# Labbeti/conette-audio-captioning

Hardware: AMD Instinct MI355X
Metric: clips_per_sec (higher is better)
Workload: dtype bf16; 1 GPU; B=64/GPU x 10 s @ 32 kHz clips, ConvNeXt encoder + beam-3 KV-cached decode (min 3 / max 20 tokens, V=5631), synthetic seeded checkpoint; batch_per_gpu=64, global_batch=64, beam_size=3, parallelism=dp1, world_size_observed=1, allreduce_of_ones=1, decode_group=2, decode_streams=2, encode_streams=1, input_batches_rotated=4

## Files before the change

conette-audio-captioning_amd/csrc/encoder.hip:

```cpp
#include <stddef.h>

#include "ctx.h"
#include <type_traits>
#include <utility>

__device__ int g_cn_nonfinite;
__device__ __forceinline__ void cn_watch_stat(float v) {
  if (!(__builtin_fabsf(v) <= 3.0e38f)) atomicAdd(&g_cn_nonfinite, 1);
}

#include "gemm2.h"
#include "mlp_rc2.h"
#include "mlp_rs16.h"
#include "mlp_sp.h"
#include "down_fused.h"
#include "enc_tags.h"

template <typename XT>
__global__ __launch_bounds__(256) void cn_stem_mfma_kernel(const float* __restrict__ in, int F, int H0, long n_pos,
                                                           const float* __restrict__ w , const float* __restrict__ bias,
                                                           const float* __restrict__ ln_w, const float* __restrict__ ln_b,
                                                           XT* __restrict__ out) {
  __shared__ __attribute__((aligned(16))) float s_p[3 * 96];
  for (int i = threadIdx.x; i < 3 * 96; i += 256) s_p[i] = i < 96 ? bias[i] : i < 192 ? ln_w[i - 96] : ln_b[i - 192];
  const int lane = threadIdx.x & 63, j = lane & 31, h = lane >> 5;
  float a[3][8];
#pragma unroll
  for (int t = 0; t < 3; ++t)
#pragma unroll
    for (int s = 0; s < 8; ++s) a[t][s] = w[(4 * (s >> 1) + 2 * h + (s & 1)) * 96 + 32 * t + cn_rc2_chan(j)];
  __syncthreads();
  const long n_tiles = (n_pos + 31) >> 5;
  const long n_waves = (long)gridDim.x * 4;
  for (long tile = (long)blockIdx.x * 4 + (threadIdx.x >> 6); tile < n_tiles; tile += n_waves) {
    const long pos = tile * 32 + j;
    const long p = pos < n_pos ? pos : n_pos - 1;
    const int wq = (int)(p % 56);
    const long tt = p / 56;
    const int hh = (int)(tt % H0);
    const int b = (int)(tt / H0);
    f32x2 xv[4];
#pragma unroll
    for (int i = 0; i < 4; ++i) {
      const int r = 4 * hh - 4 + i;
      xv[i] = f32x2{0.f, 0.f};
      if (r >= 0 && r < F) xv[i] = *(const f32x2*)(in + ((size_t)b * F + r) * CN_N_MELS + 4 * wq + 2 * h);
    }
    f32x16 acc[3];
#pragma unroll
    for (int t = 0; t < 3; ++t)
#pragma unroll
      for (int u = 0; u < 2; ++u) {
        const f32x4 b0 = *(const f32x4*)(s_p + 32 * t + 16 * u + 8 * h), b1 = *(const f32x4*)(s_p + 32 * t + 16 * u + 8 * h + 4);
#pragma unroll
        for (int e = 0; e < 4; ++e) acc[t][8 * u + e] = b0[e], acc[t][8 * u + 4 + e] = b1[e];
      }
#pragma unroll
    for (int s = 0; s < 8; ++s)
#pragma unroll
      for (int t = 0; t < 3; ++t) acc[t] = __builtin_amdgcn_mfma_f32_32x32x2f32(a[t][s], xv[s >> 1][s & 1], acc[t], 0, 0, 0);
    float sum = 0.f;
#pragma unroll
    for (int t = 0; t < 3; ++t)
#pragma unroll
      for (int r = 0; r < 16; ++r) sum += acc[t][r];
    sum += __shfl_xor(sum, 32);
    const float mean = sum * (1.0f / 96.0f);
    float v2 = 0.f;
#pragma unroll
    for (int t = 0; t < 3; ++t)
#pragma unroll
      for (int r = 0; r < 16; ++r) {
        acc[t][r] -= mean;
        v2 = fmaf(acc[t][r], acc[t][r], v2);
      }
    v2 += __shfl_xor(v2, 32);
    const float rstd = 1.0f / sqrtf(v2 * (1.0f / 96.0f) + 1e-6f);
    if (pos < n_pos) {
      XT* o = out + (size_t)pos * 96 + 8 * h;
#pragma unroll
      for (int t = 0; t < 3; ++t)
#pragma unroll
        for (int u = 0; u < 2; ++u) {
          const int ch = 32 * t + 16 * u + 8 * h;
          float v[8];
#pragma unroll
          for (int q = 0; q < 2; ++q) {
            const f32x4 lw = *(const f32x4*)(s_p + 96 + ch + 4 * q), lb = *(const f32x4*)(s_p + 192 + ch + 4 * q);
#pragma unroll
            for (int e = 0; e < 4; ++e) v[4 * q + e] = acc[t][8 * u + 4 * q + e] * rstd * lw[e] + lb[e];
          }
          if constexpr (sizeof(XT) == 2) {
            *(cn_h8<XT>*)(o + 32 * t + 16 * u) = cn_h8<XT>{cn_from_f32<XT>(v[0]), cn_from_f32<XT>(v[1]), cn_from_f32<XT>(v[2]), cn_from_f32<XT>(v[3]),
                                                          cn_from_f32<XT>(v[4]), cn_from_f32<XT>(v[5]), cn_from_f32<XT>(v[6]), cn_from_f32<XT>(v[7])};
          } else {
            *(f32x4*)(o + 32 * t + 16 * u) = f32x4{v[0], v[1], v[2], v[3]};
            *(f32x4*)(o + 32 * t + 16 * u + 4) = f32x4{v[4], v[5], v[6], v[7]};
          }
        }
    }
  }
}

__device__ unsigned long long g_dw_prof[8];
#define DW_STAMP(i)                                                   \
  if (dbg) {                                                          \
    const unsigned long long t_ = clock64();                          \
    if ((threadIdx.x & 63) == 0) atomicAdd(&g_dw_prof[i], t_ - t_prev); \
    t_prev = t_;                                                      \
  }

template <int C, int S, int TH> struct DwTile {
  static constexpr int NCHUNK = C / 4;
  static constexpr int PITCH4 = NCHUNK | 1;
  static constexpr int PITCH = PITCH4 * 4;
};

template <int... U, typename F> __device__ __forceinline__ void cn_static_for(std::integer_sequence<int, U...>, F&& f) {
  (f(std::integral_constant<int, U>{}), ...);
}
__device__ __forceinline__ void cn_dw_pin1(float& v) { asm volatile("" : "+v"(v) : : "memory"); }
template <int TH, size_t... I> __device__ __forceinline__ void cn_dw_pin(float (&acc)[TH][4], std::index_sequence<I...>) {
  (cn_dw_pin1(acc[I / 4][I % 4]), ...);
}
__device__ __forceinline__ void cn_dw_opaque(unsigned& v) { asm volatile("" : "+v"(v)); }

template <typename T, typename XT, int C, int S, int TH, bool CLAMPED = false>
__global__ __launch_bounds__((C > 384 ? 384 : C) * S) void cn_dwconv_ln_kernel(const XT* __restrict__ x, int H, int W, int tiles_h,
                                                            int tiles_w, const float* __restrict__ dw_w ,
                                                            const unsigned* __restrict__ dw_wp ,
                                                            const float* __restrict__ dw_b,
                                                            const float* __restrict__ ln_w,
                                                            const float* __restrict__ ln_b, T* __restrict__ y,
                                                            int dbg) {
  extern __shared__ __attribute__((aligned(16))) char smem_raw[];
  float* s_v = (float*)smem_raw;
  unsigned long long t_prev = dbg ? clock64() : 0;
  constexpr int NP = TH * 4;
  constexpr int CT = C > 384 ? 384 : C;
  constexpr int PITCH = DwTile<C, S, TH>::PITCH;
  const int tid = threadIdx.x;
  const int c0 = tid % CT, sidx = tid / CT;
  int bid = cn_xcd_remap(blockIdx.x, gridDim.x);
  const int tw = bid % tiles_w;
  bid /= tiles_w;
  const int th = bid % tiles_h;
  const int b = bid / tiles_h;
  const int h0 = th * TH, w0 = tw * (4 * S) + sidx * 4;

  int wcl[10];
  bool wok[10];
#pragma unroll
  for (int q = 0; q < 10; ++q) {
    const int ww = w0 - 3 + q;
    wok[q] = (ww >= 0) && (ww < W);
    wcl[q] = min(max(ww, 0), W - 1) * C;
  }
#pragma unroll 1
  for (int c = c0; c < C; c += CT) {
  float acc[TH][4];
  const float bias = dw_b[c];
#pragma unroll
  for (int a = 0; a < TH; ++a)
#pragma unroll
    for (int e = 0; e < 4; ++e) acc[a][e] = bias;
  const XT* xb = x + (size_t)b * H * W * C + c;
  const bool interior = (h0 >= 3) && (h0 + TH + 3 <= H) && (w0 >= 3) && (w0 + 4 + 3 <= W);
  if constexpr (sizeof(XT) == 2) {
    static_assert(TH % 2 == 0, "row pairs");
    cn_h2 ke[3][7], ko[3][7];
#pragma unroll
    for (int a = 0; a < 3; ++a)
#pragma unroll
      for (int j = 0; j < 7; ++j) {
        ke[a][j] = __builtin_bit_cast(cn_h2, dw_wp[(a * 7 + j) * C + c]);
        ko[a][j] = __builtin_bit_cast(cn_h2, dw_wp[(21 + a * 7 + j) * C + c]);
      }
    DW_STAMP(0)
    auto fma_pair = [&](int r, const cn_h2 (&p)[10]) {
#pragma unroll
      for (int oh = 0; oh < TH; ++oh) {
        const int i = r - oh;
        if (i < -1 || i > 6) continue;
#pragma unroll
        for (int q = 0; q < 10; ++q)
#pragma unroll
          for (int ow = 0; ow < 4; ++ow) {
            const int j = q - ow;
            if (j < 0 || j > 6) continue;
            if (i == -1) acc[oh][ow] = fmaf((float)p[q][1], (float)ke[0][j][0], acc[oh][ow]);
            else if (i == 6) acc[oh][ow] = fmaf((float)p[q][0], (float)ko[2][j][1], acc[oh][ow]);
            else if ((i & 1) == 0) acc[oh][ow] = __builtin_amdgcn_fdot2(p[q], ke[i >> 1][j], acc[oh][ow], false);
            else acc[oh][ow] = __builtin_amdgcn_fdot2(p[q], ko[i >> 1][j], acc[oh][ow], false);
          }
      }
    };
    constexpr int NPR = (TH + 6) / 2;
    if constexpr (!CLAMPED) {
      const bool left = (w0 == 0), right = (w0 + 7 > W);
      const unsigned oL = 2u * (unsigned)((left ? 0 : w0 - 3) * C + c), oM = 2u * (unsigned)(w0 * C + c);
      const unsigned oR = 2u * (unsigned)((right ? w0 + 1 : w0 + 4) * C + c);
      constexpr unsigned SEL_PAIR = 0x05040100u, SEL_ZERO = 0x0c0c0c0cu;
      const unsigned selL = left ? SEL_ZERO : SEL_PAIR, selR = right ? SEL_ZERO : SEL_PAIR;
      const char* xc = (const char*)(x + (size_t)b * H * W * C);
      const bool rows_in = (h0 >= 3) && (h0 + TH + 3 <= H);
      const unsigned rows = ((1u << min(TH + 6, H + 3 - h0)) - 1u) & ~((1u << max(0, 3 - h0)) - 1u);
      auto conv = [&](auto check_rows) {
        constexpr bool CHECK = decltype(check_rows)::value;
        auto load_row = [&](int r, unsigned (&v)[10]) {
          const int hh = h0 - 3 + r;
          if (!CHECK || ((rows >> r) & 1u)) {
            const char* xr = xc + (size_t)hh * W * C * 2;
#pragma unroll
            for (int q = 0; q < 10; ++q)
              v[q] = *(const unsigned short*)(q < 3 ? xr + (size_t)oL + q * C * 2 : q < 7 ? xr + (size_t)oM + (q - 3) * C * 2 : xr + (size_t)oR + (q - 7) * C * 2);
          } else {
#pragma unroll
            for (int q = 0; q < 10; ++q) v[q] = 0u;
          }
        };
        auto pack = [&](const unsigned (&v0)[10], const unsigned (&v1)[10], cn_h2 (&p)[10]) {
#pragma unroll
          for (int q = 0; q < 10; ++q)
            p[q] = __builtin_bit_cast(cn_h2, __builtin_amdgcn_perm(v1[q], v0[q], q < 3 ? selL : q < 7 ? SEL_PAIR : selR));
        };
        auto pin = [&]() {
          if constexpr (CHECK) cn_dw_pin(acc, std::make_index_sequence<TH * 4>{});
        };
        unsigned a0[10], a1[10], b0[10], b1[10];
        cn_h2 p[10];
        load_row(0, a0);
        load_row(1, a1);
        cn_static_for(std::make_integer_sequence<int, (NPR + 1) / 2>{}, [&](auto k) {
          constexpr int u = 2 * decltype(k)::value;
          if (u + 1 < NPR) {
            load_row(2 * u + 2, b0);
            load_row(2 * u + 3, b1);
          }
          pack(a0, a1, p);
          fma_pair(2 * u, p);
          pin();
          if (u + 2 < NPR) {
            load_row(2 * u + 4, a0);
            load_row(2 * u + 5, a1);
          }
          if (u + 1 < NPR) {
            pack(b0, b1, p);
            fma_pair(2 * (u + 1), p);
            pin();
          }
        });
      };
      if (rows_in) conv(std::false_type{});
      else conv(std::true_type{});
    } else {
#pragma unroll
      for (int u = 0; u < NPR; ++u) {
        const int hh0 = h0 - 3 + 2 * u, hh1 = hh0 + 1;
        const bool ok0 = (hh0 >= 0) && (hh0 < H), ok1 = (hh1 >= 0) && (hh1 < H);
        const XT* x0 = xb + (size_t)min(max(hh0, 0), H - 1) * W * C;
        const XT* x1 = xb + (size_t)min(max(hh1, 0), H - 1) * W * C;
        XT v0[10], v1[10];
#pragma unroll
        for (int q = 0; q < 10; ++q) v0[q] = x0[wcl[q]], v1[q] = x1[wcl[q]];
        cn_h2 p[10];
#pragma unroll
        for (int q = 0; q < 10; ++q) p[q] = cn_h2{(ok0 && wok[q]) ? v0[q] : (XT)0.f, (ok1 && wok[q]) ? v1[q] : (XT)0.f};
        fma_pair(2 * u, p);
      }
    }
  } else {
  float k[49];
#pragma unroll
  for (int i = 0; i < 49; ++i) k[i] = dw_w[i * C + c];
  DW_STAMP(0)
  auto fma_row = [&](int r, const XT (&v)[10]) {
#pragma unroll
    for (int oh = 0; oh < TH; ++oh) {
      const int i = r - oh;
      if (i < 0 || i > 6) continue;
#pragma unroll
      for (int q = 0; q < 10; ++q)
#pragma unroll
        for (int ow = 0; ow < 4; ++ow) {
          const int j = q - ow;
          if (j < 0 || j > 6) continue;
          acc[oh][ow] = fmaf((float)v[q], k[i * 7 + j], acc[oh][ow]);
        }
    }
  };
  if (interior) {
    const XT* base = xb + ((size_t)(h0 - 3) * W + (w0 - 3)) * C;
    XT va[10], vb[10];
#pragma unroll
    for (int q = 0; q < 10; ++q) va[q] = base[q * C];
#pragma unroll
    for (int r = 0; r < TH + 6; r += 2) {
      if (r + 1 < TH + 6) {
        const XT* xr = base + (size_t)(r + 1) * W * C;
#pragma unroll
        for (int q = 0; q < 10; ++q) vb[q] = xr[q * C];
      }
      fma_row(r, va);
      if (r + 2 < TH + 6) {
        const XT* xr = base + (size_t)(r + 2) * W * C;
#pragma unroll
        for (int q = 0; q < 10; ++q) va[q] = xr[q * C];
      }
      if (r + 1 < TH + 6) fma_row(r + 1, vb);
    }
  } else {
#pragma unroll
    for (int r = 0; r < TH + 6; ++r) {
      const int hh = h0 - 3 + r;
      const bool hok = (hh >= 0) && (hh < H);
      const XT* xr = xb + (size_t)min(max(hh, 0), H - 1) * W * C;
      XT v[10];
#pragma unroll
      for (int q = 0; q < 10; ++q) v[q] = xr[wcl[q]];
#pragma unroll
      for (int q = 0; q < 10; ++q) v[q] = (hok && wok[q]) ? v[q] : (XT)0.f;
      fma_row(r, v);
    }
  }
  }
#pragma unroll
  for (int oh = 0; oh < TH; ++oh)
#pragma unroll
    for (int ow = 0; ow < 4; ++ow) s_v[((sidx * NP) + oh * 4 + ow) * PITCH + c] = acc[oh][ow];
  DW_STAMP(1)
  }
  __syncthreads();
  DW_STAMP(2)

  constexpr int NPOS = NP * S, NT = CT * S, PARTS = NT / NPOS, NCHUNK = C / 4, CPT = NCHUNK / PARTS;
  static_assert(NT % NPOS == 0 && NCHUNK % PARTS == 0, "LayerNorm thread mapping");
  float* s_ps = s_v + NPOS * PITCH;
  float* s_mean = s_ps + NPOS * PARTS;
  float* s_rstd = s_mean + NPOS;
  {
    const int pos = tid % NPOS, part = tid / NPOS;
    const float* row = s_v + pos * PITCH + part * 4;
    f32x4 seg[CPT];
    float sum = 0.f;
#pragma unroll
    for (int i = 0; i < CPT; ++i) {
      seg[i] = *(const f32x4*)(row + i * PARTS * 4);
      sum += (seg[i][0] + seg[i][1]) + (seg[i][2] + seg[i][3]);
    }
    s_ps[part * NPOS + pos] = sum;
    __syncthreads();
    float mean = 0.f;
#pragma unroll
    for (int j = 0; j < PARTS; ++j) mean += s_ps[j * NPOS + pos];
    mean *= (1.0f / C);
    float sq = 0.f;
#pragma unroll
    for (int i = 0; i < CPT; ++i)
#pragma unroll
      for (int e = 0; e < 4; ++e) {
        const float d = seg[i][e] - mean;
        sq = fmaf(d, d, sq);
      }
    __syncthreads();
    s_ps[part * NPOS + pos] = sq;
    __syncthreads();
    if (part == 0) {
      float var = 0.f;
#pragma unroll
      for (int j = 0; j < PARTS; ++j) var += s_ps[j * NPOS + pos];
      s_mean[pos] = mean;
      s_rstd[pos] = 1.0f / sqrtf(var * (1.0f / C) + 1e-6f);
      cn_watch_stat(var);
    }
    __syncthreads();
  }
  DW_STAMP(3)
  constexpr int C8 = C / 8;
  static_assert(NT % C8 == 0, "a thread keeps its 8 channels over all its items: the LN affine is loaded once");
  const int c8 = (tid % C8) * 8;
  const f32x4 lw0 = *(const f32x4*)(ln_w + c8), lw1 = *(const f32x4*)(ln_w + c8 + 4);
  const f32x4 lb0 = *(const f32x4*)(ln_b + c8), lb1 = *(const f32x4*)(ln_b + c8 + 4);
  for (int item = tid; item < NPOS * C8; item += NT) {
    const int pos = item / C8;
    const int ps = pos / NP, oh = (pos % NP) >> 2, ow = pos & 3;
    const int h = h0 + oh, w = tw * (4 * S) + ps * 4 + ow;
    if (h >= H || w >= W) continue;
    const float mean = s_mean[pos], rstd = s_rstd[pos];
    const f32x4 v0 = *(const f32x4*)(s_v + pos * PITCH + c8), v1 = *(const f32x4*)(s_v + pos * PITCH + c8 + 4);
    T* dst = y + (((size_t)b * H + h) * W + w) * C + c8;
    float o[8];
#pragma unroll
    for (int i = 0; i < 8; ++i) o[i] = ((i < 4 ? v0[i] : v1[i - 4]) - mean) * rstd * (i < 4 ? lw0[i] : lw1[i - 4]) + (i < 4 ? lb0[i] : lb1[i - 4]);
    cn_store8(dst, o);
  }
  DW_STAMP(4)
}

extern "C" int conette_debug_g2prof(unsigned long long* out16, int reset) {
  if (out16) CN_HIP(hipMemcpyFromSymbol(out16, HIP_SYMBOL(g_g2_prof), 128));
  if (reset) {
    unsigned long long z[16] = {0};
    CN_HIP(hipMemcpyToSymbol(HIP_SYMBOL(g_g2_prof), z, 128));
  }
// ... 253 lines not shown
      q1 = fmaf(a1[i] - m1, a1[i] - m1, q1);
    }
    q0 = cn_wave_sum_dpp(q0);
    q1 = cn_wave_sum_dpp(q1);
    if (lane == 0) {
      s_mean[p0] = m0;
      s_rstd[p0] = 1.0f / sqrtf(q0 * (1.0f / C) + 1e-6f);
      s_mean[p1] = m1;
      s_rstd[p1] = 1.0f / sqrtf(q1 * (1.0f / C) + 1e-6f);
      cn_watch_stat(q0 + q1);
    }
  }
  __syncthreads();
  constexpr int C8 = C / 8;
  static_assert(CT % C8 == 0, "a thread keeps its 8 channels over all its items: the LN affine is loaded once");
  const int c8 = (tid % C8) * 8;
  const f32x4 lw0 = *(const f32x4*)(ln_w + c8), lw1 = *(const f32x4*)(ln_w + c8 + 4);
  const f32x4 lb0 = *(const f32x4*)(ln_b + c8), lb1 = *(const f32x4*)(ln_b + c8 + 4);
  for (int item = tid; item < NPOS * C8; item += CT) {
    const int pos = item / C8;
    const int h = h0 + pos / WW, w = pos % WW;
    if (h >= H) continue;
    const float mean = s_mean[pos], rstd = s_rstd[pos];
    const f32x4 v0 = *(const f32x4*)(s_v + pos * PITCH + c8), v1 = *(const f32x4*)(s_v + pos * PITCH + c8 + 4);
    T* dst = y + (((size_t)b * H + h) * WW + w) * C + c8;
    float o[8];
#pragma unroll
    for (int i = 0; i < 8; ++i) o[i] = ((i < 4 ? v0[i] : v1[i - 4]) - mean) * rstd * (i < 4 ? lw0[i] : lw1[i - 4]) + (i < 4 ? lb0[i] : lb1[i - 4]);
    cn_store8(dst, o);
  }
}

#ifndef CN_DW96_S
#define CN_DW96_S 2
#endif
#ifndef CN_DW96_TH
#define CN_DW96_TH 12
#endif
#ifndef CN_DW192_S
#define CN_DW192_S 1
#endif
#ifndef CN_DW192_TH
#define CN_DW192_TH 12
#endif
#ifndef CN_FW_SPLIT
#define CN_FW_SPLIT 2
#endif
#ifndef CN_FW_TH
#define CN_FW_TH 4
#endif
template <typename T, typename XT, int C, int WW, int TH, int SPLIT = 1>
static int launch_dwconv_fw(const XT* x, int B, int H, const CnBlockW& bw, T* y, hipStream_t s) {
  const int tiles_h = cn_cdiv(H, TH);
  const size_t smem = ((size_t)TH * WW * (C + 4) + 2 * TH * WW) * sizeof(float);
  CN_TRY(cn_configure_lds((const void*)cn_dwconv_ln_fw_kernel<T, XT, C, WW, TH, SPLIT>, (int)smem));
  hipLaunchKernelGGL((cn_dwconv_ln_fw_kernel<T, XT, C, WW, TH, SPLIT>), dim3((unsigned)(B * tiles_h)), dim3(C * SPLIT > 384 ? 768 : 384), smem, s, x, H,
                     tiles_h, bw.dw_w, bw.dw_wp, bw.dw_b, bw.ln_w, bw.ln_b, y);
  CN_LAUNCH_CHECK();
  return CN_OK;
}

template <typename T, typename XT, int C>
__global__ __launch_bounds__(256) void cn_ln_patchify_kernel(const XT* __restrict__ x, int H, int W, long n_pos,
                                                             const float* __restrict__ ln_w,
                                                             const float* __restrict__ ln_b, T* __restrict__ p) {
  constexpr int PER = C > 192 ? 2 : 1;
  constexpr int LANES = C / 4 / PER;
  constexpr int SLOTS = LANES <= 32 ? 2 : 1;
  constexpr int PPW = 4;
  const int lane = threadIdx.x & 63;
  const int sl = SLOTS == 2 ? lane >> 5 : 0, ll = SLOTS == 2 ? lane & 31 : lane;
  const bool act = ll < LANES;
  const long pos0 = ((long)blockIdx.x * 4 + (threadIdx.x >> 6)) * (PPW * SLOTS);
  if (pos0 >= n_pos) return;
  const int H2 = H / 2, W2 = W / 2;
  f32x4 v[PPW][PER];
#pragma unroll
  for (int u = 0; u < PPW; ++u) {
    const long pos = min(pos0 + u * SLOTS + sl, n_pos - 1);
#pragma unroll
    for (int i = 0; i < PER; ++i)
      v[u][i] = act ? cn_ld4(x + (size_t)pos * C + 4 * (ll + LANES * i)) : f32x4{0.f, 0.f, 0.f, 0.f};
  }
  f32x4 gw[PER], gb[PER];
#pragma unroll
  for (int i = 0; i < PER; ++i) {
    gw[i] = act ? *(const f32x4*)(ln_w + 4 * (ll + LANES * i)) : f32x4{0.f, 0.f, 0.f, 0.f};
    gb[i] = act ? *(const f32x4*)(ln_b + 4 * (ll + LANES * i)) : f32x4{0.f, 0.f, 0.f, 0.f};
  }
  auto group_sum = [&](float s) {
    s = cn_sum8_dpp(s);
    s += cn_dpp<0x140>(s);
    s += __shfl_xor(s, 16);
    if (SLOTS == 1) s += __shfl_xor(s, 32);
    return s;
  };
#pragma unroll
  for (int u = 0; u < PPW; ++u) {
    const long pos = pos0 + u * SLOTS + sl;
    float s = 0.f;
#pragma unroll
    for (int i = 0; i < PER; ++i) s += (v[u][i][0] + v[u][i][1]) + (v[u][i][2] + v[u][i][3]);
    const float mean = group_sum(s) * (1.0f / C);
    float s2 = 0.f;
#pragma unroll
    for (int i = 0; i < PER; ++i)
#pragma unroll
      for (int e = 0; e < 4; ++e) {
        const float d = act ? v[u][i][e] - mean : 0.f;
        s2 = fmaf(d, d, s2);
      }
    const float rstd = 1.0f / sqrtf(group_sum(s2) * (1.0f / C) + 1e-6f);
    if (pos >= n_pos || !act) continue;
    if (ll == 0) cn_watch_stat(rstd);
    const int w = (int)(pos % W);
    const long t = pos / W;
    const int h = (int)(t % H);
    const int b = (int)(t / H);
    if (h >= 2 * H2 || w >= 2 * W2) continue;
    T* o = p + ((((size_t)b * H2 + (h >> 1)) * W2 + (w >> 1)) * 4 + ((h & 1) * 2 + (w & 1))) * C;
#pragma unroll
    for (int i = 0; i < PER; ++i) {
      const int cc = 4 * (ll + LANES * i);
      cn_store4(o + cc, (v[u][i][0] - mean) * rstd * gw[i][0] + gb[i][0], (v[u][i][1] - mean) * rstd * gw[i][1] + gb[i][1],
                (v[u][i][2] - mean) * rstd * gw[i][2] + gb[i][2], (v[u][i][3] - mean) * rstd * gw[i][3] + gb[i][3]);
    }
  }
}

template <typename T, typename XT>
__global__ __launch_bounds__(256) void cn_frame_mean_kernel(const XT* __restrict__ x, int W, int C,
                                                            float* __restrict__ fe, T* __restrict__ fe_t) {
  const size_t bt = blockIdx.x;
  bool bad = false;
  for (int c = threadIdx.x; c < C; c += 256) {
    float s = 0.f;
    for (int w = 0; w < W; ++w) s += cn_ld1(x + (bt * W + w) * C + c);
    const float m = s / (float)W;
    bad |= !(__builtin_fabsf(m) <= 3.0e38f);
    fe[bt * C + c] = m;
    if (fe_t) fe_t[bt * C + c] = cn_from_f32<T>(m);
  }
  if (__syncthreads_or(bad ? 1 : 0) && threadIdx.x == 0) atomicAdd(&g_cn_nonfinite, 1);
}

template <typename T>
__global__ __launch_bounds__(256) void cn_clip_pool_ln_kernel(const float* __restrict__ fe, int Tn,
                                                              const float* __restrict__ ln_w,
                                                              const float* __restrict__ ln_b, T* __restrict__ out) {
  __shared__ float s_red[8];
  const int b = blockIdx.x, tid = threadIdx.x;
  float v[3];
  float s = 0.f;
#pragma unroll
  for (int i = 0; i < 3; ++i) {
    const int c = tid + 256 * i;
    float mx = -INFINITY, sm = 0.f;
    const float* col = fe + (size_t)b * Tn * CN_FEAT + c;
    int t = 0;
    for (; t + 8 <= Tn; t += 8) {
      float a[8];
#pragma unroll
      for (int u = 0; u < 8; ++u) a[u] = col[(size_t)(t + u) * CN_FEAT];
#pragma unroll
      for (int u = 0; u < 8; ++u) {
        mx = fmaxf(mx, a[u]);
        sm += a[u];
      }
    }
    for (; t < Tn; ++t) {
      const float a = col[(size_t)t * CN_FEAT];
      mx = fmaxf(mx, a);
      sm += a;
    }
    v[i] = mx + sm / (float)Tn;
    s += v[i];
  }
  s = cn_wave_sum(s);
  if ((tid & 63) == 0) s_red[tid >> 6] = s;
  __syncthreads();
  const float mean = (s_red[0] + s_red[1] + s_red[2] + s_red[3]) * (1.0f / CN_FEAT);
  float s2 = 0.f;
#pragma unroll
  for (int i = 0; i < 3; ++i) {
    const float d = v[i] - mean;
    s2 = fmaf(d, d, s2);
  }
  s2 = cn_wave_sum(s2);
  if ((tid & 63) == 0) s_red[4 + (tid >> 6)] = s2;
  __syncthreads();
  const float rstd = 1.0f / sqrtf((s_red[4] + s_red[5] + s_red[6] + s_red[7]) * (1.0f / CN_FEAT) + 1e-6f);
#pragma unroll
  for (int i = 0; i < 3; ++i) {
    const int c = tid + 256 * i;
    out[(size_t)b * CN_FEAT + c] = cn_from_f32<T>((v[i] - mean) * rstd * ln_w[c] + ln_b[c]);
  }
}

#ifndef CN_SP_NW96
#define CN_SP_NW96 12
#define CN_SP_NST96 4
#endif

struct EncGeom {
  int F, H[4], W[4];
};
static EncGeom enc_geom(int L) {
  EncGeom g;
  g.F = L / CN_HOP + 1;
  g.H[0] = (g.F + 8 - 4) / 4 + 1;
  g.W[0] = 56;
  for (int i = 1; i < 4; ++i) {
    g.H[i] = g.H[i - 1] / 2;
    g.W[i] = g.W[i - 1] / 2;
  }
  return g;
}

extern "C" int32_t conette_num_frames(int32_t n_samples) { return n_samples / CN_HOP + 1; }
extern "C" int32_t conette_num_audio_frames(int32_t n_samples) { return enc_geom(n_samples).H[3]; }

struct EncWs {
  float* logmel;
  void* x;
  void* y;
  void* h;
  void* fe_t;
  void* clip_t;
  size_t total;
};
static EncWs enc_ws(const conette_ctx* ctx, int B, int L, char* base) {
  const EncGeom g = enc_geom(L);
  const size_t es = ctx->esize;
  const size_t n0 = (size_t)B * g.H[0] * g.W[0] * 96;
  EncWs w;
  size_t off = 0;
  auto take = [&](size_t bytes) {
    char* p = base ? base + off : nullptr;
    off += cn_align(bytes);
    return p;
  };
  w.logmel = (float*)take((size_t)B * g.F * CN_N_MELS * 4);
  w.x = take((n0 + 32 * 96) * 4);
  w.y = take((n0 + 32 * 96) * es);
  w.h = take(n0 * 4 * es);
  w.fe_t = take((size_t)B * g.H[3] * CN_FEAT * es);
  w.clip_t = take((size_t)B * CN_FEAT * es);
  w.total = off;
  return w;
}

extern "C" size_t conette_encode_workspace_bytes(const conette_ctx* ctx, int32_t batch, int32_t n_samples) {
  return enc_ws(ctx, batch, n_samples, nullptr).total;
}

template <typename T, typename XT>
static int dwconv_dispatch(int C, const XT* x, int B, int H, int W, const CnBlockW& bw, T* y, hipStream_t s) {
  switch (C) {
    case 96: return launch_dwconv<T, XT, 96, CN_DW96_S, sizeof(XT) == 2 ? CN_DW96_TH : 8>(x, B, H, W, bw, y, s);
    case 192: return launch_dwconv<T, XT, 192, CN_DW192_S, sizeof(XT) == 2 ? CN_DW192_TH : 8>(x, B, H, W, bw, y, s);
    case 384:
      if (W == 14) return launch_dwconv_fw<T, XT, 384, 14, CN_FW_TH, CN_FW_SPLIT>(x, B, H, bw, y, s);
      return launch_dwconv<T, XT, 384, 1, 4>(x, B, H, W, bw, y, s);
    case 768:
      if (W == 7) return launch_dwconv_fw<T, XT, 768, 7, 4>(x, B, H, bw, y, s);
      return launch_dwconv<T, XT, 768, 1, 4>(x, B, H, W, bw, y, s);
  }
  cn_set_error("dwconv: unsupported C=%d", C);
  return CN_ERR_ARG;
}

static int tap_copy(float* dst, const float* src, size_t n, hipStream_t s) {
  if (dst) CN_HIP(hipMemcpyAsync(dst, src, n * sizeof(float), hipMemcpyDeviceToDevice, s));
  return CN_OK;
}
static __global__ void cn_tap_widen_kernel(const half_t* __restrict__ src, float* __restrict__ dst, size_t n) {
  for (size_t i = (size_t)blockIdx.x * blockDim.x + threadIdx.x; i < n; i += (size_t)gridDim.x * blockDim.x) dst[i] = (float)src[i];
}
static int tap_copy(float* dst, const half_t* src, size_t n, hipStream_t s) {
  if (dst) {
    hipLaunchKernelGGL(cn_tap_widen_kernel, dim3((unsigned)((n + 255) / 256 < 4096 ? (n + 255) / 256 : 4096)), dim3(256), 0, s, src, dst, n);
    CN_LAUNCH_CHECK();
  }
  return CN_OK;
}

template <typename T, typename XT>
static int encode_impl(conette_ctx* ctx, const float* wave, int B, int L, float* frame_embs, float* clip_probs,
                       const conette_encode_taps* taps, char* wsp, hipStream_t s) {
  const EncGeom g = enc_geom(L);
  EncWs ws = enc_ws(ctx, B, L, wsp);
  T* y = (T*)ws.y;
  T* hbuf = (T*)ws.h;
  XT* const wsx = (XT*)ws.x;
  {
    CnProfScope ps(ctx, CONETTE_PROF_FRONTEND, s);
    CN_TRY(cn_frontend(ctx, wave, B, L, ws.logmel, s));
  }
  if (taps) CN_TRY(tap_copy(taps->logmel, ws.logmel, (size_t)B * g.F * CN_N_MELS, s));
  {
    const long n_pos = (long)B * g.H[0] * g.W[0];
    CnProfScope ps(ctx, CONETTE_PROF_STEM, s);
    const long n_tiles = (n_pos + 31) / 32;
    const unsigned grid = (unsigned)std::min<long>((n_tiles + 3) / 4, 8L * ctx->n_cu);
    hipLaunchKernelGGL((cn_stem_mfma_kernel<XT>), dim3(grid), dim3(256), 0, s, ws.logmel, g.F, g.H[0], n_pos, ctx->stem_w, ctx->stem_b,
                       ctx->stem_ln_w, ctx->stem_ln_b, wsx);
    CN_LAUNCH_CHECK();
    if (taps) CN_TRY(tap_copy(taps->stem, wsx, (size_t)n_pos * 96, s));
  }
  XT* xc = wsx;
  int blk = 0;
  for (int st = 0; st < 4; ++st) {
    const int C = CN_DIMS[st], H = g.H[st], W = g.W[st];
    const long P = (long)B * H * W;
    if (st > 0) {
      const int Cp = CN_DIMS[st - 1], Hp = g.H[st - 1], Wp = g.W[st - 1];
      const long n_in = (long)B * Hp * Wp;
      const CnDownW& dw = ctx->down[st - 1];
      CnProfScope ps(ctx, CONETTE_PROF_DOWNSAMPLE, s);
      bool fused_down = false;
      if constexpr (CnIsH16<T>::value) if (Cp <= 192 && dw.fused != nullptr) {
        XT* xo = xc == wsx ? (XT*)ws.h : wsx;
        const int nb = ctx->n_cu - ctx->enc_reserved_cus;
        if (Cp == 96) CN_TRY((cn_launch_down_fused<96, 8, T, XT>(xc, B, Hp, Wp, dw.fused, xo, nb, s)));
        else CN_TRY((cn_launch_down_fused_ring<192, 4, 4, 3, T, XT>(xc, B, Hp, Wp, dw.fused, xo, nb, s)));
        xc = xo;
        if (taps) CN_TRY(tap_copy(taps->down[st], xc, (size_t)P * C, s));
        fused_down = true;
      }
      if (!fused_down) {
      const int ppb = Cp == 96 ? 32 : 16;
      const dim3 pg((unsigned)((n_in + ppb - 1) / ppb));
      if (Cp == 96)
        hipLaunchKernelGGL((cn_ln_patchify_kernel<T, XT, 96>), pg, dim3(256), 0, s, xc, Hp, Wp, n_in, dw.ln_w, dw.ln_b, y);
      else if (Cp == 192)
        hipLaunchKernelGGL((cn_ln_patchify_kernel<T, XT, 192>), pg, dim3(256), 0, s, xc, Hp, Wp, n_in, dw.ln_w, dw.ln_b, y);
      else
        hipLaunchKernelGGL((cn_ln_patchify_kernel<T, XT, 384>), pg, dim3(256), 0, s, xc, Hp, Wp, n_in, dw.ln_w, dw.ln_b, y);
      CN_LAUNCH_CHECK();
      EpiBiasAct<XT, ACT_NONE> epi{dw.bias, wsx, C, ACT_NONE};
      CN_TRY(cn_mm(y, 4 * Cp, (const T*)dw.w, 4 * Cp, (int)P, C, 4 * Cp, epi, s));
      xc = wsx;
      if (taps) CN_TRY(tap_copy(taps->down[st], xc, (size_t)P * C, s));
      }
    }
    for (int b = 0; b < CN_DEPTHS[st]; ++b, ++blk) {
      const CnBlockW& bw = ctx->blocks[blk];
      {
        CnProfScope ps(ctx, CONETTE_PROF_DWCONV_LN, s);
        CN_TRY((dwconv_dispatch<T, XT>(C, xc, B, H, W, bw, y, s)));
      }
      bool fused = false;
      if constexpr (std::is_same<T, sp16_t>::value) {
        if (bw.mlp_sp != nullptr && C <= 192) {
          CnProfScope ps(ctx, CONETTE_PROF_PW1_GEMM, s);
          const int nb = ctx->n_cu - ctx->enc_reserved_cus;
          if (C == 96) CN_TRY((cn_launch_mlp_sp_ring<96, CN_SP_NW96, CN_SP_NST96>(y, bw.mlp_sp, xc, (int)P, nb, s)));
          else CN_TRY((cn_launch_mlp_sp_ring<192, 8, 3>(y, bw.mlp_sp, xc, (int)P, nb, s)));
          fused = true;
        }
      }
      if constexpr (CnIsH16<T>::value) if (!fused) {
        if (bw.mlp_stream != nullptr && C <= 384) {
          CnProfScope ps(ctx, CONETTE_PROF_PW1_GEMM, s);
          const T* wsm = (const T*)bw.mlp_stream;
          if (C == 96) CN_TRY((cn_launch_mlp_rc2_resident<96, 12, 1>(y, wsm, xc, (int)P, ctx->n_cu - ctx->enc_reserved_cus, s)));
          else if (C == 192) CN_TRY((cn_launch_mlp_rc2_ring<192, 8, CN_RC2_NCK(192), CN_RC2_NCK(192) == 2 ? 3 : 5>(y, wsm, xc, (int)P, ctx->n_cu - ctx->enc_reserved_cus, s)));
          else CN_TRY((cn_launch_mlp_rs16<384, 4, 3, 8>(y, wsm, xc, (int)P, ctx->n_cu - ctx->enc_reserved_cus, s)));
          fused = true;
        }
      }
      if (!fused) {
        {
          CnProfScope ps(ctx, CONETTE_PROF_PW1_GEMM, s);
          constexpr int kAct = CnGeluAct<T>::value;
          EpiBiasAct<T, kAct> e1{bw.b1, hbuf, 4 * C, kAct};
          CN_TRY(cn_mm(y, C, (const T*)bw.w1, C, (int)P, 4 * C, C, e1, s));
        }
        {
          CnProfScope ps(ctx, CONETTE_PROF_PW2_GEMM, s);
          EpiResidT<XT> e2{bw.b2, bw.scale, xc, xc, C};
          CN_TRY(cn_mm(hbuf, 4 * C, (const T*)bw.w2, 4 * C, (int)P, C, 4 * C, e2, s));
        }
      }
      if (taps && b == 0) CN_TRY(tap_copy(taps->stage_block0[st], xc, (size_t)P * C, s));
      if (taps && taps->struct_bytes >= offsetof(conette_encode_taps, block) + (size_t)(blk + 1) * sizeof(float*))
        CN_TRY(tap_copy(taps->block[blk], xc, (size_t)P * C, s));
    }
    if (taps) CN_TRY(tap_copy(taps->stage[st], xc, (size_t)P * C, s));
  }
  const int Tn = g.H[3];
  CnProfScope ps_heads(ctx, CONETTE_PROF_HEADS, s);
  hipLaunchKernelGGL((cn_frame_mean_kernel<T, XT>), dim3((unsigned)(B * Tn)), dim3(256), 0, s, xc, g.W[3], CN_FEAT,
                     frame_embs, (T*)nullptr);
  CN_LAUNCH_CHECK();
  if (clip_probs) {
    hipLaunchKernelGGL((cn_clip_pool_ln_kernel<T>), dim3((unsigned)B), dim3(256), 0, s, frame_embs, Tn, ctx->norm_w,
                       ctx->norm_b, (T*)ws.clip_t);
    CN_LAUNCH_CHECK();
    EpiBiasAct<float> eh{ctx->head_b, clip_probs, CN_N_TAGS, ACT_SIGMOID};
    CN_TRY(cn_mm((const T*)ws.clip_t, CN_FEAT, (const T*)ctx->head_w, CN_FEAT, B, CN_N_TAGS, CN_FEAT, eh, s));
  }
  return CN_OK;
}

extern "C" int conette_encode_nonfinite(conette_ctx* ctx, void* stream, int32_t* count) {
  if (!ctx || !count) {
    cn_set_error("encode_nonfinite: bad argument");
    return CN_ERR_ARG;
  }
  hipStream_t s = (hipStream_t)stream;
  int32_t host = 0;
  CN_HIP(hipMemcpyFromSymbolAsync(&host, HIP_SYMBOL(g_cn_nonfinite), sizeof(host), 0, hipMemcpyDeviceToHost, s));
  CN_HIP(hipStreamSynchronize(s));
  if (host != 0) {
    const int32_t zero = 0;
    CN_HIP(hipMemcpyToSymbolAsync(HIP_SYMBOL(g_cn_nonfinite), &zero, sizeof(zero), 0, hipMemcpyHostToDevice, s));
    CN_HIP(hipStreamSynchronize(s));
  }
  *count = host;
  return CN_OK;
}

extern "C" int conette_frontend_logmel(conette_ctx* ctx, const float* wave, int32_t batch, int32_t n_samples,
                                       float* out, void* stream) {
  if (!ctx || !wave || !out || batch <= 0) {
    cn_set_error("frontend_logmel: bad argument");
    return CN_ERR_ARG;
  }
  if (ctx->no_encoder) {
    cn_set_error("frontend_logmel: decoder-only context (created without preprocessor.encoder.* tensors)");
    return CN_ERR_ARG;
  }
  return cn_frontend(ctx, wave, batch, n_samples, out, (hipStream_t)stream);
}

extern "C" int conette_encode(conette_ctx* ctx, const float* wave, int32_t batch, int32_t n_samples,
                              float* frame_embs, float* clip_probs, const conette_encode_taps* taps, void* workspace,
                              size_t workspace_bytes, void* stream) {
  if (conette_num_audio_frames(n_samples) < 1) {
    cn_set_error("encode: n_samples=%d is too short: the encoder's three 2x downsamplings need >= 7680 samples "
                 "(0.24 s at 32 kHz) to leave one audio frame", n_samples);
    return CN_ERR_ARG;
  }
  if (!ctx || !wave || !frame_embs || !workspace || batch <= 0) {
    cn_set_error("encode: bad argument");
    return CN_ERR_ARG;
  }
  if (ctx->no_encoder) {
    cn_set_error("encode: decoder-only context (created without preprocessor.encoder.* tensors: a BaselinePLM-layout checkpoint "
                 "takes precomputed frame embeddings)");
    return CN_ERR_ARG;
  }
  if (taps && taps->struct_bytes < offsetof(conette_encode_taps, block)) {
    cn_set_error("encode: conette_encode_taps.struct_bytes = %zu is smaller than the version-1 members (%zu): set it to "
                 "sizeof(conette_encode_taps)", taps->struct_bytes, offsetof(conette_encode_taps, block));
    return CN_ERR_ARG;
  }
  const size_t need = conette_encode_workspace_bytes(ctx, batch, n_samples);
  if (workspace_bytes < need) {
    cn_set_error("encode: workspace %zu < %zu", workspace_bytes, need);
    return CN_ERR_WORKSPACE;
  }
  switch (ctx->cfg.precision) {
    case CONETTE_PREC_BF16:
      return encode_impl<bf16_t, half_t>(ctx, wave, batch, n_samples, frame_embs, clip_probs, taps, (char*)workspace, (hipStream_t)stream);
    case CONETTE_PREC_F16:
      return encode_impl<half_t, half_t>(ctx, wave, batch, n_samples, frame_embs, clip_probs, taps, (char*)workspace, (hipStream_t)stream);
    case CONETTE_PREC_F16X2:
      return encode_impl<sp16_t, float>(ctx, wave, batch, n_samples, frame_embs, clip_probs, taps, (char*)workspace, (hipStream_t)stream);
    default:
      return encode_impl<float, float>(ctx, wave, batch, n_samples, frame_embs, clip_probs, taps, (char*)workspace, (hipStream_t)stream);
  }
}

extern "C" size_t conette_tag_frames_workspace_bytes(const conette_ctx* ctx, int32_t batch, int32_t t_audio) {
  if (!ctx || batch < 0 || t_audio < 0) return 0;
  return cn_align((size_t)batch * t_audio * CN_FEAT * ctx->esize);
}

template <typename T>
static int tag_frames_impl(conette_ctx* ctx, const float* frame_embs, const int32_t* frame_lens, int B, int Tn, int window,
                           float* frame_probs, T* z, hipStream_t s) {
  const dim3 grid((unsigned)cn_cdiv(Tn, CN_TAG_TT), (unsigned)B);
  hipLaunchKernelGGL((cn_window_pool_ln_kernel<T>), grid, dim3(256), 0, s, frame_embs, frame_lens, Tn, (window - 1) / 2, window / 2,
                     ctx->norm_w, ctx->norm_b, z);
  CN_LAUNCH_CHECK();
  EpiBiasAct<float> eh{ctx->head_b, frame_probs, CN_N_TAGS, ACT_SIGMOID};
  CN_TRY(cn_mm((const T*)z, CN_FEAT, (const T*)ctx->head_w, CN_FEAT, B * Tn, CN_N_TAGS, CN_FEAT, eh, s));
  hipLaunchKernelGGL(cn_tag_zero_rows_kernel, grid, dim3(256), 0, s, frame_probs, frame_lens, Tn, CN_N_TAGS);
  CN_LAUNCH_CHECK();
  return CN_OK;
}

extern "C" int conette_tag_frames(conette_ctx* ctx, const float* frame_embs, const int32_t* frame_lens, int32_t batch,
                                  int32_t t_audio, int32_t window, float* frame_probs, void* workspace, size_t workspace_bytes,
                                  void* stream) {
  const char* bad = !ctx ? "ctx" : !frame_embs ? "frame_embs" : !frame_lens ? "frame_lens" : !frame_probs ? "frame_probs" : nullptr;
  if (bad) {
    cn_set_error("tag_frames: %s is NULL", bad);
    return CN_ERR_ARG;
  }
  if (ctx->no_encoder) {
    cn_set_error("tag_frames: decoder-only context (created without preprocessor.encoder.* tensors: it holds no clip head)");
    return CN_ERR_ARG;
  }
  if (batch < 0 || batch > 65535) {
    cn_set_error("tag_frames: batch=%d unsupported (0..65535)", batch);
    return CN_ERR_ARG;
  }
  if (t_audio < 0 || (int64_t)batch * t_audio > INT32_MAX / CN_FEAT) {
    cn_set_error("tag_frames: t_audio=%d unsupported (0..%d frames in the whole batch)", t_audio, INT32_MAX / CN_FEAT);
    return CN_ERR_ARG;
  }
  if (window < 1 || window > CONETTE_TAG_MAX_WINDOW) {
    cn_set_error("tag_frames: window=%d unsupported (1..%d frames)", window, CONETTE_TAG_MAX_WINDOW);
    return CN_ERR_ARG;
  }
  if (batch == 0 || t_audio == 0) return CN_OK;
  const size_t need = conette_tag_frames_workspace_bytes(ctx, batch, t_audio);
  if (!workspace) {
    cn_set_error("tag_frames: workspace is NULL");
    return CN_ERR_ARG;
  }
  if (workspace_bytes < need) {
    cn_set_error("tag_frames: workspace_bytes %zu < %zu", workspace_bytes, need);
    return CN_ERR_WORKSPACE;
  }
  hipStream_t s = (hipStream_t)stream;
  switch (ctx->cfg.precision) {
    case CONETTE_PREC_BF16: return tag_frames_impl(ctx, frame_embs, frame_lens, batch, t_audio, window, frame_probs, (bf16_t*)workspace, s);
    case CONETTE_PREC_F16: return tag_frames_impl(ctx, frame_embs, frame_lens, batch, t_audio, window, frame_probs, (half_t*)workspace, s);
    case CONETTE_PREC_F16X2: return tag_frames_impl(ctx, frame_embs, frame_lens, batch, t_audio, window, frame_probs, (sp16_t*)workspace, s);
    default: return tag_frames_impl(ctx, frame_embs, frame_lens, batch, t_audio, window, frame_probs, (float*)workspace, s);
  }
}

extern "C" int conette_tag_events(const float* frame_probs, const int32_t* frame_lens, int32_t batch, int32_t t_audio,
                                  int32_t n_tags, float on_threshold, float off_threshold, int32_t min_frames, int32_t max_gap,
                                  int32_t max_events, int32_t* spans, float* peaks, int32_t* peak_frames, int32_t* counts,
                                  void* stream) {
  const char* bad = !frame_probs ? "frame_probs" : !frame_lens ? "frame_lens" : !spans ? "spans" : !peaks ? "peaks"
                    : !peak_frames ? "peak_frames" : !counts ? "counts" : nullptr;
  if (bad) {
    cn_set_error("tag_events: %s is NULL", bad);
    return CN_ERR_ARG;
  }
  if (batch < 0 || t_audio < 0 || n_tags < 0 || (int64_t)batch * n_tags > INT32_MAX / CONETTE_TAG_MAX_EVENTS) {
    cn_set_error("tag_events: %s=%d unsupported (at least 0, batch * n_tags at most %d)", batch < 0 ? "batch" : t_audio < 0 ? "t_audio" : "n_tags",
                 batch < 0 ? batch : t_audio < 0 ? t_audio : n_tags, INT32_MAX / CONETTE_TAG_MAX_EVENTS);
    return CN_ERR_ARG;
  }
  if (!(on_threshold > 0.0f && on_threshold <= 1.0f)) {
    cn_set_error("tag_events: on_threshold=%g unsupported (finite, 0 < off_threshold <= on_threshold <= 1)", (double)on_threshold);
    return CN_ERR_ARG;
  }
  if (!(off_threshold > 0.0f && off_threshold <= on_threshold)) {
    cn_set_error("tag_events: off_threshold=%g unsupported (finite, 0 < off_threshold <= on_threshold = %g)", (double)off_threshold,
                 (double)on_threshold);
    return CN_ERR_ARG;
  }
  if (min_frames < 0 || max_gap < 0) {
    cn_set_error("tag_events: %s=%d unsupported (at least 0)", min_frames < 0 ? "min_frames" : "max_gap", min_frames < 0 ? min_frames : max_gap);
    return CN_ERR_ARG;
  }
  if (max_events < 1 || max_events > CONETTE_TAG_MAX_EVENTS) {
    cn_set_error("tag_events: max_events=%d unsupported (1..%d)", max_events, CONETTE_TAG_MAX_EVENTS);
    return CN_ERR_ARG;
  }
  const long n_seq = (long)batch * n_tags;
  if (n_seq == 0) return CN_OK;
  CnTagEventsArgs a;
  a.probs = frame_probs;
  a.lens = frame_lens;
  a.batch = batch;
  a.t_audio = t_audio;
  a.n_tags = n_tags;
  a.on = on_threshold;
  a.off = off_threshold;
  a.min_frames = min_frames;
  a.max_gap = max_gap;
  a.max_events = max_events;
  a.spans = spans;
  a.peaks = peaks;
  a.peak_frames = peak_frames;
  a.counts = counts;
  hipLaunchKernelGGL(cn_tag_events_kernel, dim3((unsigned)((n_seq + 255) / 256)), dim3(256), 0, (hipStream_t)stream, a);
  CN_LAUNCH_CHECK();
  return CN_OK;
}
```

Measured before the change: 13600 clips/s.

## Software-pipeline stem kernel loads and use 32-bit indexing with smaller grid

The stem conv+LayerNorm kernel now prefetches the next tile's log-mel rows while the current tile's MFMA and normalisation run. It clamps row indices so loads are unconditional and masks them to zero afterwards. When sizes fit, it uses unsigned 32-bit index arithmetic in place of 64-bit divisions, and the grid cap drops from 8 to 3 blocks per CU with a matching launch-bounds occupancy hint. The aim is to hide global load latency and cut integer division cost in a small, memory-bound stage, at the cost of extra registers and fewer resident waves.

```diff
diff --git a/conette-audio-captioning_amd/csrc/encoder.hip b/conette-audio-captioning_amd/csrc/encoder.hip
--- a/conette-audio-captioning_amd/csrc/encoder.hip
+++ b/conette-audio-captioning_amd/csrc/encoder.hip
@@ -16,36 +16,35 @@
 #include "down_fused.h"
 #include "enc_tags.h"
 
-template <typename XT>
-__global__ __launch_bounds__(256) void cn_stem_mfma_kernel(const float* __restrict__ in, int F, int H0, long n_pos,
-                                                           const float* __restrict__ w , const float* __restrict__ bias,
-                                                           const float* __restrict__ ln_w, const float* __restrict__ ln_b,
-                                                           XT* __restrict__ out) {
-  __shared__ __attribute__((aligned(16))) float s_p[3 * 96];
-  for (int i = threadIdx.x; i < 3 * 96; i += 256) s_p[i] = i < 96 ? bias[i] : i < 192 ? ln_w[i - 96] : ln_b[i - 192];
-  const int lane = threadIdx.x & 63, j = lane & 31, h = lane >> 5;
-  float a[3][8];
-#pragma unroll
-  for (int t = 0; t < 3; ++t)
-#pragma unroll
-    for (int s = 0; s < 8; ++s) a[t][s] = w[(4 * (s >> 1) + 2 * h + (s & 1)) * 96 + 32 * t + cn_rc2_chan(j)];
-  __syncthreads();
-  const long n_tiles = (n_pos + 31) >> 5;
-  const long n_waves = (long)gridDim.x * 4;
-  for (long tile = (long)blockIdx.x * 4 + (threadIdx.x >> 6); tile < n_tiles; tile += n_waves) {
-    const long pos = tile * 32 + j;
-    const long p = pos < n_pos ? pos : n_pos - 1;
-    const int wq = (int)(p % 56);
-    const long tt = p / 56;
-    const int hh = (int)(tt % H0);
-    const int b = (int)(tt / H0);
-    f32x2 xv[4];
-#pragma unroll
-    for (int i = 0; i < 4; ++i) {
-      const int r = 4 * hh - 4 + i;
-      xv[i] = f32x2{0.f, 0.f};
-      if (r >= 0 && r < F) xv[i] = *(const f32x2*)(in + ((size_t)b * F + r) * CN_N_MELS + 4 * wq + 2 * h);
-    }
+#ifndef CN_STEM_WAVES
+#define CN_STEM_WAVES 3
+#endif
+template <typename IT>
+__device__ __forceinline__ int cn_stem_load(const float* __restrict__ in, int F, int H0, IT n_pos, IT tile, int j, int h, f32x2 (&xv)[4]) {
+  const IT pos = tile * 32 + (IT)j;
+  const IT p = pos < n_pos ? pos : n_pos - 1;
+  const int wq = (int)(p % 56);
+  const IT tt = p / 56;
+  const int hh = (int)(tt % (IT)H0);
+  const IT b = tt / (IT)H0;
+  int ok = 0;
+#pragma unroll
+  for (int i = 0; i < 4; ++i) {
+    const int r = 4 * hh - 4 + i;
+    const int rc = r < 0 ? 0 : r < F ? r : F - 1;
+    xv[i] = *(const f32x2*)(in + (size_t)((b * (IT)F + (IT)rc) * CN_N_MELS + (IT)(4 * wq + 2 * h)));
+    if (r >= 0 && r < F) ok |= 1 << i;
+  }
+  return ok;
+}
+__device__ __forceinline__ void cn_stem_rows(const f32x2 (&xn)[4], int ok, f32x2 (&xv)[4]) {
+#pragma unroll
+  for (int i = 0; i < 4; ++i) xv[i] = (ok >> i & 1) ? xn[i] : f32x2{0.f, 0.f};
+}
+template <typename XT, typename IT, bool TESTED>
+__device__ __forceinline__ void cn_stem_tile(const float (&a)[3][8], const f32x2 (&xv)[4], const float* s_p, IT pos, IT n_pos, int h,
+                                             XT* __restrict__ out) {
+  {
     f32x16 acc[3];
 #pragma unroll
     for (int t = 0; t < 3; ++t)
@@ -76,7 +75,7 @@
       }
     v2 += __shfl_xor(v2, 32);
     const float rstd = 1.0f / sqrtf(v2 * (1.0f / 96.0f) + 1e-6f);
-    if (pos < n_pos) {
+    if (!TESTED || pos < n_pos) {
       XT* o = out + (size_t)pos * 96 + 8 * h;
 #pragma unroll
       for (int t = 0; t < 3; ++t)
@@ -100,6 +99,36 @@
         }
     }
   }
+}
+template <typename XT, typename IT>
+__global__ __launch_bounds__(256, CN_STEM_WAVES) void cn_stem_mfma_kernel(const float* __restrict__ in, int F, int H0, IT n_pos,
+                                                           const float* __restrict__ w , const float* __restrict__ bias,
+                                                           const float* __restrict__ ln_w, const float* __restrict__ ln_b,
+                                                           XT* __restrict__ out) {
+  __shared__ __attribute__((aligned(16))) float s_p[3 * 96];
+  for (int i = threadIdx.x; i < 3 * 96; i += 256) s_p[i] = i < 96 ? bias[i] : i < 192 ? ln_w[i - 96] : ln_b[i - 192];
+  const int lane = threadIdx.x & 63, j = lane & 31, h = lane >> 5;
+  float a[3][8];
+#pragma unroll
+  for (int t = 0; t < 3; ++t)
+#pragma unroll
+    for (int s = 0; s < 8; ++s) a[t][s] = w[(4 * (s >> 1) + 2 * h + (s & 1)) * 96 + 32 * t + cn_rc2_chan(j)];
+  __syncthreads();
+  const IT n_tiles = (n_pos + 31) >> 5, n_whole = n_pos >> 5;
+  const IT n_waves = (IT)gridDim.x * 4;
+  IT tile = (IT)blockIdx.x * 4 + (IT)__builtin_amdgcn_readfirstlane(threadIdx.x >> 6);
+  f32x2 xn[4], xv[4];
+  int ok = cn_stem_load<IT>(in, F, H0, n_pos, tile < n_tiles ? tile : n_tiles - 1, j, h, xn);
+  cn_stem_rows(xn, ok, xv);
+  for (; tile < n_whole; tile += n_waves) {
+    const IT nx = tile + n_waves;
+    ok = cn_stem_load<IT>(in, F, H0, n_pos, nx < n_tiles ? nx : n_tiles - 1, j, h, xn);
+    asm volatile("" : : : "memory");
+    cn_stem_tile<XT, IT, false>(a, xv, s_p, tile * 32 + (IT)j, n_pos, h, out);
+    asm volatile("" : "+v"(ok) : "v"(xn[0]), "v"(xn[1]), "v"(xn[2]), "v"(xn[3]) : "memory");
+    cn_stem_rows(xn, ok, xv);
+  }
+  if (tile < n_tiles) cn_stem_tile<XT, IT, true>(a, xv, s_p, tile * 32 + (IT)j, n_pos, h, out);
 }
 
 __device__ unsigned long long g_dw_prof[8];
@@ -959,9 +988,13 @@
     const long n_pos = (long)B * g.H[0] * g.W[0];
     CnProfScope ps(ctx, CONETTE_PROF_STEM, s);
     const long n_tiles = (n_pos + 31) / 32;
-    const unsigned grid = (unsigned)std::min<long>((n_tiles + 3) / 4, 8L * ctx->n_cu);
-    hipLaunchKernelGGL((cn_stem_mfma_kernel<XT>), dim3(grid), dim3(256), 0, s, ws.logmel, g.F, g.H[0], n_pos, ctx->stem_w, ctx->stem_b,
-                       ctx->stem_ln_w, ctx->stem_ln_b, wsx);
+    const unsigned grid = (unsigned)std::min<long>((n_tiles + 3) / 4, (long)CN_STEM_WAVES * ctx->n_cu);
+    if (n_pos * 96 + 96 < (1L << 31) && (long)B * g.F * CN_N_MELS < (1L << 31))
+      hipLaunchKernelGGL((cn_stem_mfma_kernel<XT, unsigned>), dim3(grid), dim3(256), 0, s, ws.logmel, g.F, g.H[0], (unsigned)n_pos, ctx->stem_w,
+                         ctx->stem_b, ctx->stem_ln_w, ctx->stem_ln_b, wsx);
+    else
+      hipLaunchKernelGGL((cn_stem_mfma_kernel<XT, long>), dim3(grid), dim3(256), 0, s, ws.logmel, g.F, g.H[0], n_pos, ctx->stem_w, ctx->stem_b,
+                         ctx->stem_ln_w, ctx->stem_ln_b, wsx);
     CN_LAUNCH_CHECK();
     if (taps) CN_TRY(tap_copy(taps->stem, wsx, (size_t)n_pos * 96, s));
   }
```

After: 13650 clips/s, median of 6. About the same (+0.4%).
